# learningmatter-mit/surface-sampling

Measured on AMD Instinct MI355X. Metric: MC energy-evaluations/sec (SrTiO3(001) ~250-atom slabs, 3-model PaiNN ensemble E+F incl. neighbor list), higher is better.
Workload: dtype f32 via fp16x2-split MFMA (3 products), fp32 accumulate; neighbor decisions f64; 1 GPU; SrTiO3(001) PaiNN x3, 256 batched independent chains per GPU (BASELINE configs[3]), 248-272 atoms/chain; chains_per_gpu=256, atoms_per_gpu=66503, edges_per_gpu=2747786, slots_per_gpu=2836316, models=3, streams_per_gpu=2, parallelism=one GPU, no collective

## Files before the change

surface-sampling_amd/csrc/nbr.hip:

```cpp
#include "nbr_dev.h"

namespace vssr {

__global__ void k_wrap(int n, const double *__restrict__ pos, const int *__restrict__ atom_cfg,
                       const double *__restrict__ cell, const double *__restrict__ invcell,
                       const uint8_t *__restrict__ pbc, double *__restrict__ wpos, int *__restrict__ wrap) {
    int i = blockIdx.x * blockDim.x + threadIdx.x;
    if (i >= n) return;
    wrap_atom(i, pos, atom_cfg, cell, invcell, pbc, wpos, wrap);
}

template <bool FILL, int LPC>
__global__ void __launch_bounds__(256)
k_nbr(int n, const double *__restrict__ wpos, const int *__restrict__ atom_cfg,
      const int *__restrict__ cfg_start, const double *__restrict__ cell, const double *__restrict__ invcell,
      const int *__restrict__ nimg, double rc2, int *__restrict__ deg, const int *__restrict__ row_start, float4 *__restrict__ edge,
      int *__restrict__ edge_S, long long slot_cap, unsigned long long *__restrict__ hits_buf, int hits_stride,
      const unsigned char *__restrict__ active) {
    const int i = blockIdx.x * (256 / LPC) + threadIdx.x / LPC;
    if (i >= n) return;
    nbr_row<FILL, LPC>(i, wpos, atom_cfg, cfg_start, cell, invcell, nimg, rc2, deg, row_start, edge, edge_S, slot_cap, hits_buf, hits_stride,
                       active);
}

struct ScanTile {
    int d[4], pd[4], p, real;
};
__device__ __forceinline__ ScanTile scan_tile_load(int n, const int *__restrict__ deg, int i0) {
    ScanTile s;
    if (i0 + 3 < n) {
        const int4 v = *reinterpret_cast<const int4 *>(deg + i0);
        s.d[0] = v.x; s.d[1] = v.y; s.d[2] = v.z; s.d[3] = v.w;
    } else {
#pragma unroll
        for (int u = 0; u < 4; ++u) s.d[u] = i0 + u < n ? deg[i0 + u] : 0;
    }
#pragma unroll
    for (int u = 0; u < 4; ++u) s.pd[u] = i0 + u < n ? max((s.d[u] + 3) & ~3, 8) : 0;
    s.p = s.pd[0] + s.pd[1] + s.pd[2] + s.pd[3];
    s.real = s.d[0] + s.d[1] + s.d[2] + s.d[3];
    return s;
}

__global__ void __launch_bounds__(1024)
k_scan_tiles(int n, const int *__restrict__ deg, int *__restrict__ tile_sums ) {
    __shared__ int wsum[16], wreal[16];
    const int t = threadIdx.x, lane = t & 63, w = t >> 6;
    const ScanTile s = scan_tile_load(n, deg, blockIdx.x * 4096 + 4 * t);
    const int x = wave_incl_scan_i32(s.p), xr = wave_incl_scan_i32(s.real);
    if (lane == 63) { wsum[w] = x; wreal[w] = xr; }
    __syncthreads();
    if (t == 0) {
        int a = 0, b = 0;
#pragma unroll
        for (int k = 0; k < 16; ++k) { a += wsum[k]; b += wreal[k]; }
        tile_sums[2 * blockIdx.x] = a;
        tile_sums[2 * blockIdx.x + 1] = b;
    }
}

__global__ void __launch_bounds__(1024)
k_scan_rows(int n, const int *__restrict__ deg, int *__restrict__ row_start, int *__restrict__ counters,
            long long slot_cap, const int *__restrict__ tile_sums) {
    __shared__ int wsum[16], wreal[16];
    __shared__ long long wrun[16], wrun_real[16];
    const int t = threadIdx.x, lane = t & 63, w = t >> 6, tile = blockIdx.x;
    const bool last = tile == (int)gridDim.x - 1;
    long long run = 0, run_real = 0;
    for (int k = t; k < tile; k += 1024) {
        run += tile_sums[2 * k];
        if (last) run_real += tile_sums[2 * k + 1];
    }
#pragma unroll
    for (int o = 32; o > 0; o >>= 1) {
        run += __shfl_xor(run, o);
        run_real += __shfl_xor(run_real, o);
    }
    if (lane == 0) { wrun[w] = run; wrun_real[w] = run_real; }
    const ScanTile s = scan_tile_load(n, deg, tile * 4096 + 4 * t);
    const int x = wave_incl_scan_i32(s.p);
    if (lane == 63) wsum[w] = x;
    if (!tile_sums) {
        const int xr = wave_incl_scan_i32(s.real);
        if (lane == 63) wreal[w] = xr;
    }
    __syncthreads();
    run = 0; run_real = 0;
    int woff = 0;
#pragma unroll
    for (int k = 0; k < 16; ++k) {
        run += wrun[k];
        run_real += wrun_real[k];
        if (k < w) woff += wsum[k];
    }
    const int i0 = tile * 4096 + 4 * t;
    int o = (int)(run + woff + x - s.p);
#pragma unroll
    for (int u = 0; u < 4; ++u) {
        if (i0 + u < n) row_start[i0 + u] = o;
        o += s.pd[u];
    }
    if (last && t == 0) {
        long long own = 0, own_real = 0;
        if (tile_sums) { own = tile_sums[2 * tile]; own_real = tile_sums[2 * tile + 1]; }
        else {
            for (int k = 0; k < 16; ++k) { own += wsum[k]; own_real += wreal[k]; }
        }
        const long long total = run + own, total_real = run_real + own_real;
        row_start[n] = (int)total;
        counters[0] = (int)total;
        counters[1] = (int)total_real;
        counters[2] = (total > slot_cap - 64 || total > 2147483000LL) ? 1 : 0;
    }
}

template <int LPC>
__global__ void __launch_bounds__(256)
k_rev(int n, const int *__restrict__ row_start, const float4 *__restrict__ edge,
      const int *__restrict__ edge_S, int *__restrict__ rev, const int *__restrict__ counters, ActiveView av) {
    const int i = blockIdx.x * (256 / LPC) + threadIdx.x / LPC;
    if (i >= n || counters[2] || !av.atom(i)) return;
    rev_row<LPC>(i, row_start, edge, edge_S, rev);
}

__device__ __forceinline__ void split2_f16(float x, unsigned &h, unsigned &l) {
    const _Float16 hh = (_Float16)x;
    const _Float16 ll = (_Float16)(x - (float)hh);
    h = __builtin_bit_cast(unsigned short, hh);
    l = __builtin_bit_cast(unsigned short, ll);
}
__device__ __forceinline__ size_t f16_unit(size_t slot, int kq, int piece) {
    return (slot >> 2) * 32 + (size_t)piece * 16 + (size_t)kq * 4 + (slot & 3);
}
__device__ __forceinline__ void write_f16_record(const float (&v)[5], float env, uint4 *__restrict__ tab, size_t slot, int kq,
                                                 float spare, unsigned jbits) {
    unsigned h[6], l[6];
#pragma unroll
    for (int k = 0; k < 5; ++k) split2_f16(v[k], h[k], l[k]);
    split2_f16(env, h[5], l[5]);
    auto pk = [](unsigned lo, unsigned hi) { return lo | (hi << 16); };
    const unsigned env_piece = kq == 0 ? l[5] : kq == 3 ? 0u : h[5];
    tab[f16_unit(slot, kq, 0)] = make_uint4(pk(l[0], l[1]), pk(l[2], l[3]), pk(l[4], env_piece), pk(h[0], h[1]));
    tab[f16_unit(slot, kq, 1)] = make_uint4(pk(h[2], h[3]), pk(h[4], h[4]), __float_as_uint(spare), jbits);
}

__device__ __forceinline__ float quarter_class_sum(float x) {
    x += __builtin_bit_cast(float, __builtin_amdgcn_update_dpp(0, __builtin_bit_cast(int, x), 0x124, 0xF, 0xF, true));
    x += __builtin_bit_cast(float, __builtin_amdgcn_update_dpp(0, __builtin_bit_cast(int, x), 0x128, 0xF, 0xF, true));
    const unsigned u = __float_as_uint(x);
    const auto r32 = __builtin_amdgcn_permlane32_swap(u, u, false, false);
    const float y = __uint_as_float(r32[0]) + __uint_as_float(r32[1]);
    const unsigned v = __float_as_uint(y);
    const auto r16 = __builtin_amdgcn_permlane16_swap(v, v, false, false);
    return __uint_as_float(r16[0]) + __uint_as_float(r16[1]);
}

template <int NZ>
__global__ void __launch_bounds__(64) k_edge_geom(int n_atoms, const int *__restrict__ row_start, const int *__restrict__ atom_cfg,
                            const int *__restrict__ cfg_start, const float4 *__restrict__ edge,
                            const int *__restrict__ counters, float rc, float excl_sigma, int excl_power,
                            float4 *__restrict__ erec, float *__restrict__ rho,
                            float2 *__restrict__ dist2, uint4 *__restrict__ rho16, uint4 *__restrict__ drho16,
                            const int *__restrict__ Z, const int *__restrict__ zmap, unsigned char *__restrict__ zslot,
                            float *__restrict__ e_excl, const unsigned char *__restrict__ active, float *__restrict__ l0T) {
    if (counters[2]) return;
    float tacc[NZ > 0 ? NZ : 1][4][6];
#pragma unroll
    for (int z = 0; z < (NZ > 0 ? NZ : 1); ++z)
#pragma unroll
        for (int c = 0; c < 4; ++c)
#pragma unroll
            for (int k = 0; k < 6; ++k) tacc[z][c][k] = 0.f;
    const int i = blockIdx.x;
    if (active && !active[atom_cfg[i]]) return;
    const int a0 = cfg_start[atom_cfg[i]];
// ... 71 lines not shown
            float x = __uint_as_float(r16[0]) + __uint_as_float(r16[1]);
            x += __builtin_bit_cast(float, __builtin_amdgcn_update_dpp(0, __builtin_bit_cast(int, x), 0x128, 0xF, 0xF, true));
            x += __builtin_bit_cast(float, __builtin_amdgcn_update_dpp(0, __builtin_bit_cast(int, x), 0x124, 0xF, 0xF, true));
            quart[w] = x;
        }
        const int lane = threadIdx.x, rho = lane >> 4, kq = lane & 3;
        if ((lane & 12) == 0) {
#pragma unroll
            for (int b = 0; b < NZ; ++b) {
                const int zc = rho * NZ + b, z = zc >> 2, c = zc & 3;
                float2 *dst = reinterpret_cast<float2 *>(l0T + ((size_t)i * NZ + z) * 96 + c * 24 + kq * 6);
                dst[0] = make_float2(quart[6 * b], quart[6 * b + 1]);
                dst[1] = make_float2(quart[6 * b + 2], quart[6 * b + 3]);
                dst[2] = make_float2(quart[6 * b + 4], quart[6 * b + 5]);
            }
        }
    }
}

constexpr int BSORT_N = 2048;
__device__ __forceinline__ void lds_bitonic_sort(unsigned *keys) {
    for (int k = 2; k <= BSORT_N; k <<= 1)
        for (int j = k >> 1; j > 0; j >>= 1) {
            for (int t = threadIdx.x; t < BSORT_N / 2; t += blockDim.x) {
                const int i = 2 * t - (t & (j - 1)), l = i + j;
                const unsigned a = keys[i], b2 = keys[l];
                const bool up = (i & k) == 0;
                if ((a > b2) == up) { keys[i] = b2; keys[l] = a; }
            }
            __syncthreads();
        }
}

__global__ void __launch_bounds__(256)
k_bundle_sort(const int *__restrict__ cfg_start, const int *__restrict__ row_start, const int *__restrict__ counters,
              int4 *__restrict__ bundle, const unsigned char *__restrict__ active, int sort_keys) {
    extern __shared__ int sdeg[];
    if (counters[2] || (active && !active[blockIdx.x])) return;
    const int b = blockIdx.x, a0 = cfg_start[b], n = cfg_start[b + 1] - a0;
    for (int c = threadIdx.x; c < n; c += blockDim.x) sdeg[c] = row_start[a0 + c + 1] - row_start[a0 + c];
    __syncthreads();
    if (n <= BSORT_N && sort_keys) {
        unsigned *keys = reinterpret_cast<unsigned *>(sdeg) + n;
        for (int c = threadIdx.x; c < BSORT_N; c += blockDim.x) keys[c] = c < n ? ((unsigned)(4095 - min(sdeg[c], 4095)) << 11) | (unsigned)c : 0xFFFFFFFFu;
        __syncthreads();
        lds_bitonic_sort(keys);
        for (int r = threadIdx.x; r < n; r += blockDim.x) {
            const int c = (int)(keys[r] & 2047u);
            bundle[a0 + r] = make_int4(c, row_start[a0 + c], sdeg[c], 0);
        }
        return;
    }
    for (int c = threadIdx.x; c < n; c += blockDim.x) {
        const int d = sdeg[c];
        int rank = 0;
        for (int o = 0; o < n; ++o) {
            const int od = sdeg[o];
            rank += (od > d || (od == d && o < c)) ? 1 : 0;
        }
        bundle[a0 + rank] = make_int4(c, row_start[a0 + c], d, 0);
    }
}

__global__ void __launch_bounds__(1024)
k_bundle_sort_sub(const int *__restrict__ list, const int *__restrict__ cfg_start, const int *__restrict__ row_start,
                  const float4 *__restrict__ edge, const int *__restrict__ counters, int N, int n_cfg, int chunk_max,
                  int4 *__restrict__ bundle_sub, int *__restrict__ n_entries, const unsigned char *__restrict__ active) {
    extern __shared__ int sdeg[];
    const int b = list[blockIdx.x];
    if (counters[2] || (active && !active[b])) return;
    const int a0 = cfg_start[b], n = cfg_start[b + 1] - a0;
    const int P = sub_passes(n, chunk_max), chunk = sub_chunk(n, chunk_max);
    int *len = sdeg, *first = sdeg + SUB_MAX_PASSES * n;
    __shared__ int cnt[SUB_MAX_PASSES];
    if (threadIdx.x < SUB_MAX_PASSES) cnt[threadIdx.x] = 0;
    __syncthreads();
    const int lane = threadIdx.x & 15;
    for (int c = threadIdx.x >> 4; c < n; c += blockDim.x >> 4) {
        const int rs = row_start[a0 + c], re = row_start[a0 + c + 1];
        int below[SUB_MAX_PASSES];
#pragma unroll
        for (int p = 0; p < SUB_MAX_PASSES; ++p) below[p] = 0;
        for (int e = rs + lane; e < re; e += 16) {
            const int j = __float_as_int(edge[e].w);
            if (j < 0) continue;
            const int jl = j - a0;
#pragma unroll
            for (int p = 0; p < SUB_MAX_PASSES; ++p) below[p] += (p + 1 >= P || jl < (p + 1) * chunk) ? 1 : 0;
        }
#pragma unroll
        for (int p = 0; p < SUB_MAX_PASSES; ++p) {
            int x = below[p];
            x += __shfl_xor(x, 1); x += __shfl_xor(x, 2); x += __shfl_xor(x, 4); x += __shfl_xor(x, 8);
            below[p] = x;
        }
        if (lane == 0) {
            int kprev = 0;
            for (int p = 0; p < P; ++p) {
                const int k = below[p];
                const bool any = k > kprev;
                const int f = kprev & ~3, last = p + 1 < P ? min((k + 3) & ~3, re - rs) : re - rs;
                len[p * n + c] = any ? last - f : 0;
                first[p * n + c] = f;
                if (any && p > 0) atomicAdd(&cnt[p], 1);
                kprev = k;
            }
        }
    }
    __syncthreads();
    if (threadIdx.x >= 1 && threadIdx.x < SUB_MAX_PASSES) n_entries[(size_t)(threadIdx.x - 1) * n_cfg + b] = cnt[threadIdx.x];
    unsigned *keys = reinterpret_cast<unsigned *>(sdeg + 2 * SUB_MAX_PASSES * n);
    for (int p = 0; p < P; ++p) {
        const int *lp = len + p * n;
        __syncthreads();
        for (int c = threadIdx.x; c < BSORT_N; c += blockDim.x) keys[c] = c < n ? ((unsigned)(4095 - min(lp[c], 4095)) << 11) | (unsigned)c : 0xFFFFFFFFu;
        __syncthreads();
        lds_bitonic_sort(keys);
        for (int r = threadIdx.x; r < n; r += blockDim.x) {
            const int c = (int)(keys[r] & 2047u);
            bundle_sub[(size_t)p * N + a0 + r] = make_int4(c, row_start[a0 + c] + first[p * n + c], lp[c], 0);
        }
    }
}

int build_neighbors(vssr_handle *h, double cutoff) {
    const int n = h->n_atoms;
    hipStream_t st = h->stream;
    if (h->d_wpos.ensure(sizeof(double) * 3 * n) || h->d_wrap.ensure(sizeof(int) * 3 * n) ||
        h->d_deg.ensure(sizeof(int) * n) || h->d_row_start.ensure(sizeof(int) * (n + 1)) ||
        h->d_counters.ensure(sizeof(int) * 4) || h->d_tile_sums.ensure(sizeof(int) * 2 * ((size_t)n / 4096 + 1)))
        return set_err(h, VSSR_E_NOMEM, "neighbor buffers: out of device memory");
    if (h->slot_cap < (int64_t)n * h->cap_per_atom + 64) h->slot_cap = (int64_t)n * h->cap_per_atom + 64;
    if (h->d_edge.ensure(sizeof(float4) * h->slot_cap) || h->d_edge_S.ensure(sizeof(int) * h->slot_cap) ||
        h->d_rev.ensure(sizeof(int) * h->slot_cap))
        return set_err(h, VSSR_E_NOMEM, "edge buffers: out of device memory");
    unsigned long long *hits_buf = nullptr;
    const int hits_stride = (h->max_cfg_atoms + 63) & ~63;
    if (h->max_images <= 64 && (size_t)n * hits_stride * 8 <= ((size_t)1 << 30) &&
        !h->d_hits.ensure((size_t)n * hits_stride * 8))
        hits_buf = h->d_hits.as<unsigned long long>();
    h->prof.begin(KC_NBR, st);
    dim3 blk(128), grd((n + 127) / 128);
    const int lpc_rev = h->kind != Kind::PAINN ? 16 : 32;
    dim3 wblk(256);
    auto grid_for = [&](int lpc) { return dim3((n + 256 / lpc - 1) / (256 / lpc)); };
#define NBR_ARGS(FILLING) n, h->d_wpos.as<double>(), h->d_atom_cfg.as<int>(), h->d_cfg_start.as<int>(), h->d_cell.as<double>(),          \
        h->d_invcell.as<double>(), h->d_nimg.as<int>(), cutoff * cutoff, h->d_deg.as<int>(),                                            \
        (FILLING) ? h->d_row_start.as<int>() : (const int *)nullptr, (FILLING) ? h->d_edge.as<float4>() : (float4 *)nullptr,            \
        (FILLING) ? h->d_edge_S.as<int>() : (int *)nullptr, (FILLING) ? (long long)h->slot_cap : (long long)0, hits_buf, hits_stride,   \
        h->active_mask
    hipLaunchKernelGGL(k_wrap, grd, blk, 0, st, n, h->d_pos.as<double>(), h->d_atom_cfg.as<int>(),
                       h->d_cell.as<double>(), h->d_invcell.as<double>(), h->d_pbc.as<uint8_t>(),
                       h->d_wpos.as<double>(), h->d_wrap.as<int>());
    hipLaunchKernelGGL((k_nbr<false, 16>), grid_for(16), wblk, 0, st, NBR_ARGS(false));
    const int n_tiles = n > 0 ? (n + 4095) / 4096 : 1;
    if (n_tiles > 1)
        hipLaunchKernelGGL(k_scan_tiles, dim3(n_tiles), dim3(1024), 0, st, n, h->d_deg.as<int>(), h->d_tile_sums.as<int>());
    hipLaunchKernelGGL(k_scan_rows, dim3(n_tiles), dim3(1024), 0, st, n, h->d_deg.as<int>(),
                       h->d_row_start.as<int>(), h->d_counters.as<int>(), (long long)h->slot_cap,
                       n_tiles > 1 ? h->d_tile_sums.as<int>() : (const int *)nullptr);
    hipLaunchKernelGGL((k_nbr<true, 16>), grid_for(16), wblk, 0, st, NBR_ARGS(true));
#undef NBR_ARGS
    const ActiveView rev_av{h->active_mask, h->d_atom_cfg.as<int>()};
#define REV_ARGS n, h->d_row_start.as<int>(), h->d_edge.as<float4>(), h->d_edge_S.as<int>(), h->d_rev.as<int>(), h->d_counters.as<int>(), rev_av
    if (lpc_rev == 16) hipLaunchKernelGGL(k_rev<16>, grid_for(16), wblk, 0, st, REV_ARGS);
    else hipLaunchKernelGGL(k_rev<32>, grid_for(32), wblk, 0, st, REV_ARGS);
#undef REV_ARGS
    if (h->kind == Kind::PAINN && !h->painn_general) {
        const int nzf = (h->l0_enabled && h->l0_nz >= 1 && h->l0_nz <= 4) ? h->l0_nz : 0;
        const bool want_f32 = h->l0_enabled && nzf == 0;
        if ((want_f32 && (h->d_erec.ensure(sizeof(float4) * h->slot_cap) || h->d_rho.ensure(sizeof(float) * 24 * h->slot_cap))) ||
            h->d_dist.ensure(sizeof(float2) * h->slot_cap) ||
            h->d_rho16.ensure(sizeof(uint4) * 8 * h->slot_cap) || h->d_drho16.ensure(sizeof(uint4) * 8 * h->slot_cap) ||
            h->d_zslot.ensure((size_t)h->slot_cap) || h->d_bundle.ensure(sizeof(int4) * (size_t)n) ||
            h->d_excl.ensure(sizeof(float) * (size_t)n))
            return set_err(h, VSSR_E_NOMEM, "edge geometry tables: out of device memory");
        const void *tabs[2] = {h->d_rho16.as<uint4>(), h->d_drho16.as<uint4>()};
        bool cleared = h->zero_entry_cap == h->slot_cap;
        for (int k = 0; k < 2; ++k) cleared = cleared && h->zero_entry_tab[k] == tabs[k];
        if (!cleared) {
            VSSR_HIP(h, hipMemsetAsync(h->d_rho16.as<uint4>() + 32 * (size_t)((h->slot_cap >> 2) - 1), 0, 32 * sizeof(uint4), st));
            VSSR_HIP(h, hipMemsetAsync(h->d_drho16.as<uint4>() + 32 * (size_t)((h->slot_cap >> 2) - 1), 0, 32 * sizeof(uint4), st));
            h->zero_entry_cap = h->slot_cap;
            for (int k = 0; k < 2; ++k) h->zero_entry_tab[k] = tabs[k];
        }
        if (nzf && h->d_l0T.ensure(sizeof(float) * (size_t)n * nzf * 96))
            return set_err(h, VSSR_E_NOMEM, "layer-0 factorisation buffers: out of device memory");
        h->l0T_by_geom = nzf > 0;
#define LAUNCH_GEOM(NZ)                                                                                                          \
        hipLaunchKernelGGL(k_edge_geom<NZ>, dim3(n), dim3(64), 0, st, n, h->d_row_start.as<int>(), h->d_atom_cfg.as<int>(),      \
                           h->d_cfg_start.as<int>(), h->d_edge.as<float4>(), h->d_counters.as<int>(), h->cutoff,               \
                           h->excl_sigma, h->excl_power, want_f32 ? h->d_erec.as<float4>() : (float4 *)nullptr,                \
                           want_f32 ? h->d_rho.as<float>() : (float *)nullptr, h->d_dist.as<float2>(), h->d_rho16.as<uint4>(), \
                           h->d_drho16.as<uint4>(), h->d_Z.as<int>(), h->d_zmap.as<int>(), h->d_zslot.as<unsigned char>(),     \
                           h->d_excl.as<float>(), h->active_mask, nzf ? h->d_l0T.as<float>() : (float *)nullptr)
        switch (nzf) {
            case 1: LAUNCH_GEOM(1); break;
            case 2: LAUNCH_GEOM(2); break;
            case 3: LAUNCH_GEOM(3); break;
            case 4: LAUNCH_GEOM(4); break;
            default: LAUNCH_GEOM(0); break;
        }
#undef LAUNCH_GEOM
        if ((size_t)h->max_cfg_atoms * sizeof(int) <= 48 * 1024) {
            const int sort_keys = h->max_cfg_atoms > 512 && h->max_cfg_atoms <= BSORT_N;
            hipLaunchKernelGGL(k_bundle_sort, dim3(h->n_cfg), dim3(256),
                               (size_t)h->max_cfg_atoms * sizeof(int) + (sort_keys ? BSORT_N * sizeof(unsigned) : 0), st,
                               h->d_cfg_start.as<int>(), h->d_row_start.as<int>(), h->d_counters.as<int>(),
                               h->d_bundle.as<int4>(), h->active_mask, sort_keys);
            auto sub_tables = [&](vssr::DevBuf &buf, const int *list, int n_list, int max_atoms, int chunk) -> int {
                if (sub_passes(max_atoms, chunk) > SUB_MAX_PASSES) return set_err(h, VSSR_E_BADARG, "neighbor sub-range too small for this chain");
                if (buf.ensure(sizeof(int4) * SUB_MAX_PASSES * (size_t)n + sizeof(int) * (SUB_MAX_PASSES - 1) * (size_t)h->n_cfg))
                    return set_err(h, VSSR_E_NOMEM, "bundle tables: out of device memory");
                hipLaunchKernelGGL(k_bundle_sort_sub, dim3(n_list), dim3(1024),
                                   2 * SUB_MAX_PASSES * (size_t)max_atoms * sizeof(int) + BSORT_N * sizeof(unsigned), st, list,
                                   h->d_cfg_start.as<int>(), h->d_row_start.as<int>(), h->d_edge.as<float4>(), h->d_counters.as<int>(), n, h->n_cfg,
                                   chunk, buf.as<int4>(), reinterpret_cast<int *>(buf.as<int4>() + SUB_MAX_PASSES * (size_t)n), h->active_mask);
                return VSSR_OK;
            };
            if (h->fwd_two_pass && h->n_class[EDGE_CLASS_FS4] > 0) {
                int off = 0;
                for (int c = 0; c < EDGE_CLASS_FS4; ++c) off += h->n_class[c];
                const int rc2 = sub_tables(h->d_bundle_sub, h->d_class_list.as<int>() + off, h->n_class[EDGE_CLASS_FS4], h->max_class_atoms[EDGE_CLASS_FS4],
                                           h->sub_chunk_fwd ? h->sub_chunk_fwd : sub_chunk_max(h->fwd_two_pass));
                if (rc2) return rc2;
            }
            if (h->n_bclass[EDGE_BCLASS_FS16P] > 0) {
                int off = 0;
                for (int c = 0; c < EDGE_MFMA_CLASSES; ++c) off += h->n_class[c];
                for (int c = 0; c < EDGE_BCLASS_FS16P; ++c) off += h->n_bclass[c];
                const int rc2 = sub_tables(h->d_bundle_subb, h->d_class_list.as<int>() + off, h->n_bclass[EDGE_BCLASS_FS16P],
                                           h->max_bclass_atoms[EDGE_BCLASS_FS16P], h->sub_chunk_bwd ? h->sub_chunk_bwd : sub_chunk_max_bwd());
                if (rc2) return rc2;
            }
        }
    }
    h->prof.end(st);
    VSSR_HIP(h, hipMemcpyAsync(h->h_counters, h->d_counters.as<int>(), sizeof(int) * 4,
                               hipMemcpyDeviceToHost, st));
    return VSSR_OK;
}

}
```

surface-sampling_amd/csrc/nbr_dev.h:

```cpp
#ifndef VSSR_NBR_DEV_H
#define VSSR_NBR_DEV_H
#include "vssr_internal.h"

namespace vssr {

__device__ inline int pack_shift(int s0, int s1, int s2) {
    return ((s0 + 128) & 255) | (((s1 + 128) & 255) << 8) | (((s2 + 128) & 255) << 16);
}
__device__ inline void unpack_shift(int p, int &s0, int &s1, int &s2) {
    s0 = (p & 255) - 128;
    s1 = ((p >> 8) & 255) - 128;
    s2 = ((p >> 16) & 255) - 128;
}

__device__ __forceinline__ void wrap_atom(int i, const double *__restrict__ pos, const int *__restrict__ atom_cfg,
                                          const double *__restrict__ cell, const double *__restrict__ invcell,
                                          const uint8_t *__restrict__ pbc, double *__restrict__ wpos, int *__restrict__ wrap) {
    int c = atom_cfg[i];
    const double *C = cell + 9 * c, *I = invcell + 9 * c;
    double p[3] = {pos[3 * i], pos[3 * i + 1], pos[3 * i + 2]};
    double q[3] = {p[0], p[1], p[2]};
    for (int a = 0; a < 3; ++a) {
        int w = 0;
        if (pbc[3 * c + a]) {
            double f = I[3 * a] * p[0] + I[3 * a + 1] * p[1] + I[3 * a + 2] * p[2];
            w = (int)floor(f);
            q[0] -= w * C[3 * a];
            q[1] -= w * C[3 * a + 1];
            q[2] -= w * C[3 * a + 2];
        }
        wrap[3 * i + a] = w;
    }
    wpos[3 * i] = q[0];
    wpos[3 * i + 1] = q[1];
    wpos[3 * i + 2] = q[2];
}

template <int LPC>
__device__ __forceinline__ int group_excl_scan(int v, int &total) {
    if constexpr (LPC == 64) {
        const int x = wave_incl_scan_i32(v);
        total = __builtin_amdgcn_readlane(x, 63);
        return x - v;
    } else {
        static_assert(LPC == 16 || LPC == 32, "a wave, half a wave or one 16-lane row per centre");
        int x = v;
        x += __builtin_amdgcn_update_dpp(0, x, 0x111, 0xF, 0xF, true);
        x += __builtin_amdgcn_update_dpp(0, x, 0x112, 0xF, 0xF, true);
        x += __builtin_amdgcn_update_dpp(0, x, 0x114, 0xF, 0xF, true);
        x += __builtin_amdgcn_update_dpp(0, x, 0x118, 0xF, 0xF, true);
        if constexpr (LPC == 32) x += __builtin_amdgcn_update_dpp(0, x, 0x142, 0xA, 0xF, false);
        total = __shfl(x, (threadIdx.x & 63) | (LPC - 1));
        return x - v;
    }
}

template <bool FILL, int LPC>
__device__ __forceinline__ void nbr_row(int i, const double *__restrict__ wpos, const int *__restrict__ atom_cfg,
      const int *__restrict__ cfg_start, const double *__restrict__ cell, const double *__restrict__ invcell,
      const int *__restrict__ nimg, double rc2, int *__restrict__ deg, const int *__restrict__ row_start, float4 *__restrict__ edge,
      int *__restrict__ edge_S, long long slot_cap, unsigned long long *__restrict__ hits_buf, int hits_stride,
      const unsigned char *__restrict__ active) {
    const int lane = threadIdx.x & (LPC - 1);
    const int c = atom_cfg[i];
    if (active && !active[c]) {
        if (!FILL && lane == 0) deg[i] = 0;
        return;
    }
    const int a0 = cfg_start[c], a1 = cfg_start[c + 1];
    const double *C = cell + 9 * c;
    const int n0 = nimg[3 * c], n1 = nimg[3 * c + 1], n2 = nimg[3 * c + 2];
    const double C0 = C[0], C1 = C[1], C2 = C[2], C3 = C[3], C4 = C[4], C5 = C[5], C6 = C[6], C7 = C[7], C8 = C[8];
    const double px = wpos[3 * i], py = wpos[3 * i + 1], pz = wpos[3 * i + 2];
    const double *I = invcell + 9 * c;
    const double I0 = I[0], I1 = I[1], I2 = I[2], I3 = I[3], I4 = I[4], I5 = I[5], I6 = I[6], I7 = I[7], I8 = I[8];
    const double rcut = sqrt(rc2);
    const double wd0 = rcut * sqrt(I0 * I0 + I1 * I1 + I2 * I2) * (1.0 + 1e-9) + 1e-9;
    const double wd1 = rcut * sqrt(I3 * I3 + I4 * I4 + I5 * I5) * (1.0 + 1e-9) + 1e-9;
    const double wd2 = rcut * sqrt(I6 * I6 + I7 * I7 + I8 * I8) * (1.0 + 1e-9) + 1e-9;
    long long base = FILL ? (long long)row_start[i] : 0;
    int run = 0;
    for (int j0 = a0; j0 < a1; j0 += LPC) {
        const int j = j0 + lane;
        const bool have = j < a1;
        double bx = 0, by = 0, bz = 0;
        if (have) { bx = wpos[3 * j] - px; by = wpos[3 * j + 1] - py; bz = wpos[3 * j + 2] - pz; }
        int cnt = 0;
        unsigned long long hits = 0ull;
        unsigned long long *hslot = hits_buf ? hits_buf + (size_t)i * hits_stride + (j - a0) : nullptr;
        if (FILL && hslot) {
            if (have) {
                hits = *hslot;
                cnt = __builtin_popcountll(hits);
            }
        } else if (have) {
            const double f0 = I0 * bx + I1 * by + I2 * bz, f1 = I3 * bx + I4 * by + I5 * bz, f2 = I6 * bx + I7 * by + I8 * bz;
            const int lo0 = n0 ? max(-n0, (int)ceil(-wd0 - f0)) : 0, hi0 = n0 ? min(n0, (int)floor(wd0 - f0)) : 0;
            const int lo1 = n1 ? max(-n1, (int)ceil(-wd1 - f1)) : 0, hi1 = n1 ? min(n1, (int)floor(wd1 - f1)) : 0;
            const int lo2 = n2 ? max(-n2, (int)ceil(-wd2 - f2)) : 0, hi2 = n2 ? min(n2, (int)floor(wd2 - f2)) : 0;
            const int iw1 = 2 * n1 + 1, iw2 = 2 * n2 + 1;
            for (int s0 = lo0; s0 <= hi0; ++s0)
                for (int s1 = lo1; s1 <= hi1; ++s1)
                    for (int s2 = lo2; s2 <= hi2; ++s2) {
                        const int img = ((s0 + n0) * iw1 + (s1 + n1)) * iw2 + (s2 + n2);
                        if (i == j && s0 == 0 && s1 == 0 && s2 == 0) continue;
                        double rx = bx + s0 * C0 + s1 * C3 + s2 * C6;
                        double ry = by + s0 * C1 + s1 * C4 + s2 * C7;
                        double rz = bz + s0 * C2 + s1 * C5 + s2 * C8;
                        double d2 = rx * rx + ry * ry + rz * rz;
                        if (d2 <= rc2 && d2 > 0.0) {
                            ++cnt;
                            if (img < 64) hits |= 1ull << img;
                        }
                    }
            if (!FILL && hslot) *hslot = hits;
        }
        int total;
        const int off = group_excl_scan<LPC>(cnt, total);
        if (FILL && cnt > 0) {
            long long slot = base + run + off;
            const int w1 = 2 * n1 + 1, w2 = 2 * n2 + 1;
            if ((2 * n0 + 1) * w1 * w2 <= 64) {
                while (hits) {
                    const int img = __builtin_ctzll(hits);
                    hits &= hits - 1;
                    const int s0 = img / (w1 * w2) - n0, s1 = (img / w2) % w1 - n1, s2 = img % w2 - n2;
                    const double rx = bx + s0 * C0 + s1 * C3 + s2 * C6;
                    const double ry = by + s0 * C1 + s1 * C4 + s2 * C7;
                    const double rz = bz + s0 * C2 + s1 * C5 + s2 * C8;
                    if (slot < slot_cap) {
                        edge[slot] = make_float4((float)rx, (float)ry, (float)rz, __int_as_float(j));
                        edge_S[slot] = pack_shift(s0, s1, s2);
                    }
                    ++slot;
                }
            } else {
                for (int s0 = -n0; s0 <= n0; ++s0)
                    for (int s1 = -n1; s1 <= n1; ++s1)
                        for (int s2 = -n2; s2 <= n2; ++s2) {
                            if (i == j && s0 == 0 && s1 == 0 && s2 == 0) continue;
                            double rx = bx + s0 * C0 + s1 * C3 + s2 * C6;
                            double ry = by + s0 * C1 + s1 * C4 + s2 * C7;
                            double rz = bz + s0 * C2 + s1 * C5 + s2 * C8;
                            double d2 = rx * rx + ry * ry + rz * rz;
                            if (d2 > rc2 || d2 <= 0.0) continue;
                            if (slot < slot_cap) {
                                edge[slot] = make_float4((float)rx, (float)ry, (float)rz, __int_as_float(j));
                                edge_S[slot] = pack_shift(s0, s1, s2);
                            }
                            ++slot;
                        }
            }
        }
        run += total;
    }
    if (FILL) {
        const int padded = max((run + 3) & ~3, 8);
        const long long slot = base + run + lane;
        if (lane < padded - run && slot < slot_cap) {
            edge[slot] = make_float4(0.f, 0.f, 0.f, __int_as_float(-1));
            edge_S[slot] = pack_shift(0, 0, 0);
        }
    } else if (lane == 0) {
        deg[i] = run;
    }
}

template <int LPC>
__device__ __forceinline__ void rev_row(int i, const int *__restrict__ row_start, const float4 *__restrict__ edge,
                                        const int *__restrict__ edge_S, int *__restrict__ rev) {
    const int lane = threadIdx.x & (LPC - 1);
    for (int e = row_start[i] + lane; e < row_start[i + 1]; e += LPC) {
        int j = __float_as_int(edge[e].w);
        int found = -1;
        if (j >= 0) {
            int s0, s1, s2;
            unpack_shift(edge_S[e], s0, s1, s2);
            const int want = pack_shift(-s0, -s1, -s2);
            int lo = row_start[j], hi = row_start[j + 1];
            const int row_end = hi;
            while (lo < hi) {
                const int mid = (lo + hi) >> 1;
                const int jm = __float_as_int(edge[mid].w);
                if (jm >= 0 && jm < i) lo = mid + 1; else hi = mid;
            }
            for (int e2 = lo; e2 < row_end && __float_as_int(edge[e2].w) == i; ++e2)
                if (edge_S[e2] == want) {
                    found = e2;
                    break;
                }
        }
        rev[e] = found;
    }
}

}
#endif
```

surface-sampling_amd/csrc/vssr_internal.h:

```cpp
#pragma once

#include <hip/hip_runtime.h>

#include <cstdint>
#include <cstdio>
#include <cstdlib>
#include <cstring>
#include <memory>
#include <string>
#include <utility>
#include <vector>

#include "../../include/vssr_eval.h"

namespace vssr {

constexpr int F = 128;
constexpr int F3 = 3 * F;
constexpr int MAX_LAYERS = 4;
constexpr int MAX_MODELS = 8;
constexpr int RB_MAX = 24;
constexpr int NODE_TILE = 8;
constexpr int L0_MAX_SPECIES = 8;

// ... 162 lines not shown
    OwnedStream &operator=(const OwnedStream &) = delete;
    ~OwnedStream() { if (s) (void)hipStreamDestroy(s); }
    operator hipStream_t() const { return s; }
};
struct PinnedInts {
    int *p = nullptr;
    PinnedInts() = default;
    PinnedInts(const PinnedInts &) = delete;
    PinnedInts &operator=(const PinnedInts &) = delete;
    ~PinnedInts() { if (p) (void)hipHostFree(p); }
    operator int *() const { return p; }
};

enum KernelClass {
    KC_NBR = 0,
    KC_EMBED,
    KC_MSG_MLP,
    KC_EDGE_FWD,
    KC_UPDATE_FWD,
    KC_READOUT,
    KC_UPDATE_BWD,
    KC_EDGE_BWD,
    KC_MSG_MLP_BWD,
    KC_FINALIZE,
    KC_ANALYTIC,
    KC_L0_FWD,
    KC_L0_BWD,
    KC_NEB_PROJECT,
    KC_NEB_STEP,
    KC_COUNT
};
extern const char *const kKernelClassNames[KC_COUNT];

struct Profiler {
    bool enabled = false;
    struct Rec { int kc; hipEvent_t a, b; };
    std::vector<Rec> pending;
    std::vector<hipEvent_t> pool;
    int64_t launches[KC_COUNT] = {0};
    double total_ms[KC_COUNT] = {0};
    hipEvent_t get_event();
    void begin(int kc, hipStream_t s);
    void end(hipStream_t s);
    void collect();
    void reset();
    Profiler() = default;
    Profiler(const Profiler &) = delete;
    Profiler &operator=(const Profiler &) = delete;
    ~Profiler();
};

struct GmmFit {
    int cov_type = 0;
    int init = 0;
    int max_iter = 100, n_init = 1;
    double tol = 1e-3, reg_covar = 1e-6;
    uint64_t seed = 0;
    bool device_ready = false, fitted = false;
    int64_t n = 0, cap = 0;
    DevBuf rows;
    double *x() const { return rows.as<double>(); }
    std::vector<double> i_means, i_weights, i_prec;
    std::vector<int> i_labels;
    bool has_means = false, has_weights = false, has_prec = false, has_labels = false;
    DevBuf resp, labels, lbpart, status, flags;
    DevBuf part_s, part_q, part_n, nk, means, avg_x2, w, cov, part_cov, chol_w, chol_y, centers, assign_part;
    DevBuf b_w, b_means, b_cov, b_P, b_c, b_kc, b_mask;
};

struct Cluster {
    int n_components = 0, whiten = 1, d_clu = 3, d_pad = 3;
    bool pca_done = false;
    int64_t n_pts = 0;
    DevBuf mean, denom, part_sum, part_cov, cov, evec, eval, comp, comp_t, ev, ratio, jac, xr;
    DevBuf pts;
    DevBuf cen[2], siz[2], cid[2];
    DevBuf nn, flag, blk, rec, counters;
};

enum class Kind : int {
    NONE = 0,
    PAINN = 1,
    TERSOFF = 2,
    EAM = 3,
    SW = 4,
    GMM = 5,
    GMM_FIT = 6,
    CLUSTER = 7,
    PAIR = 8,
    VASHISHTA = 9,
    COUNT
};
constexpr unsigned kind_bit(Kind k) { return 1u << (int)k; }
constexpr unsigned KINDS_EVAL = kind_bit(Kind::PAINN) | kind_bit(Kind::TERSOFF) | kind_bit(Kind::EAM) | kind_bit(Kind::SW) |
                                kind_bit(Kind::PAIR) | kind_bit(Kind::VASHISHTA);

}

struct vssr_handle {
    vssr::Kind kind = vssr::Kind::NONE;
    vssr_eam_grid eam_grid = {0, 0, 0.0, 0.0, 0.0};
    int eam_nel = 0, eam_fs = 0;
    bool eam_adp = false;
    double vash_r0max = 0.0;
    int device = 0;
    vssr::OwnedStream stream;
    std::string err;
    vssr::Profiler prof;

    int edge_impl = 1;
    int max_cfg_atoms = 0;
    vssr::DevBuf d_chain_class, d_class_list;
    int n_class[5] = {0, 0, 0, 0, 0}, max_class_atoms[5] = {0, 0, 0, 0, 0};
    int n_bclass[5] = {0, 0, 0, 0, 0}, max_bclass_atoms[5] = {0, 0, 0, 0, 0};
    int fs16_max_atoms = -1, fs8_max_atoms = -1;
    int max_images = 0;

    int n_models = 0, n_rbf = 20, num_conv = 3, n_embed = 100, readout_hidden = 64;
    int feat_dim = vssr::F;
    bool painn_general = false;
    float cutoff = 5.f;
    int excl_vol = 1, excl_power = 12;
    float excl_sigma = 1.5f;
    double units_per_ev = 1.0;
    bool has_offset = false;
    double offset_const = 0.0;

    vssr::DevBuf weights;
    vssr::DevBuf wd16;
    vssr::DevBuf node16;
    vssr::DevBuf model_table;
    vssr::DevBuf offset_per_z;

    int n_types = 0;
    double pot_cutoff = 0;
    bool ew_on = false;
    double ew_g = 0, ew_kcut = 0, ew_q[8] = {0, 0, 0, 0, 0, 0, 0, 0};
    int ew_stride = 0;
    vssr::DevBuf d_ew_S;
    vssr::DevBuf pot_params;

    bool batch_valid = false, ran = false;
    int n_cfg = 0, n_atoms = 0;
    std::vector<int> h_n_atoms, h_cfg_start;
    vssr::DevBuf d_pos, d_wpos, d_wrap, d_Z, d_atom_cfg, d_cfg_start, d_cell, d_invcell, d_nimg, d_pbc;
    vssr::DevBuf d_deg, d_row_start, d_edge, d_edge_S, d_rev, d_counters, d_tile_sums;
    vssr::DevBuf d_erec, d_rho, d_dist, d_rho16, d_drho16, d_zslot, d_bundle, d_excl;
    vssr::DevBuf d_bundle_sub;
    int bwd_multi_pass = 1;
    int sub_chunk_fwd = 0, sub_chunk_bwd = 0;
    vssr::DevBuf d_bundle_subb;
    int fwd_two_pass = 16;
    vssr::DevBuf d_hits;
    int l0_enabled = 1, l0_nz = 0;
    bool l0_used = false;
    vssr::DevBuf d_l0A, d_l0At;
    vssr::DevBuf d_zmap, d_zlist;
    vssr::DevBuf d_l0T, d_l0Q;
    vssr::DevBuf d_opt_state, d_opt_vec, d_bfgs_q, d_bfgs_b, d_fixed, d_relax_steps, d_relax_conv, d_active;
    const unsigned char *active_mask = nullptr;
    int relax_regrows = 0;
    long long relax_lockstep = 0;
    int relax_compactions = 0;
    vssr::DevBuf d_cmp;
    vssr::DevBuf d_cm;
    long long relax_chain_evals = 0;
    int traj_interval = 0, traj_records = 0, traj_B = 0, traj_N = 0;
    vssr::DevBuf d_traj_pos, d_traj_f, d_traj_e, d_traj_n;
    bool graph_partial = false;
    bool l0T_by_geom = false;
    int64_t zero_entry_cap = -1;
    const void *zero_entry_tab[2] = {nullptr, nullptr};
    int cap_per_atom = 64;
    int cm_cap_per_atom = 0;
    int cg_driver = 0;
    int cg_last_driver = 0;
    bool cap_tight = false;
    vssr::DevBuf d_md_vel;
    vssr::DevBuf d_md_aux;
    bool md_vel_valid = false;
    int md_driver = 0;
    int md_last_driver = 0;
    vssr::DevBuf d_vib;
    vssr::DevBuf d_neb;
    uint32_t last_want = 0;
    int64_t slot_cap = 0;
    vssr::PinnedInts h_counters;

    vssr::DevBuf d_state;
    vssr::StateView sv;
    vssr::DevBuf d_gbar;
    vssr::DevBuf d_upd_save;
    vssr::DevBuf d_gpart;
    int debug_keep = 0;
    int upd_save = 0;
    vssr::DevBuf d_energy, d_energy_std, d_energy_models, d_forces, d_forces_std, d_e_atoms;
    vssr::DevBuf d_energy64;
    vssr::DevBuf d_pot_e, d_pot_ea, d_pot_f;
    vssr::DevBuf d_sat, d_sat_out;
    std::vector<unsigned> h_sat;
    bool h_sat_valid = false;
    vssr::DevBuf d_stress;

    int gmm_K = 0, gmm_D = 0, gmm_Dp = 0;
    double gmm_log2pi = 0.0;
    vssr::DevBuf d_gmm_P;
    vssr::DevBuf d_gmm_c;
    vssr::DevBuf d_gmm_kc;
    vssr::DevBuf d_gmm_mask;
    vssr::DevBuf d_gmm_x, d_gmm_lp, d_gmm_nll, d_gmm_sys, d_gmm_start;
    std::unique_ptr<vssr::GmmFit> fit;
    std::unique_ptr<vssr::Cluster> clu;
};

namespace vssr {

int set_err(vssr_handle *h, int code, const char *fmt, ...);
#define VSSR_HIP(h, expr)                                                                    \
    do {                                                                                     \
        hipError_t _e = (expr);                                                              \
        if (_e != hipSuccess)                                                                \
            return vssr::set_err(h, VSSR_E_DEVICE, "%s failed: %s (%s:%d)", #expr,          \
                                 hipGetErrorString(_e), __FILE__, __LINE__);                 \
    } while (0)

int check_kind(vssr_handle *h, unsigned served, const char *func);
int device_in_range(vssr_handle *h, int device);
int open_device(vssr_handle *h, int device);
void publish_create_error(const vssr_handle *h);
template <class Init>
int create_handle(Kind kind, int device, vssr_handle **out, Init init, bool range_check = true) {
    vssr_handle *h = new vssr_handle();
    h->kind = kind;
    int rc = range_check ? device_in_range(h, device) : VSSR_OK;
    if (!rc) rc = open_device(h, device);
    if (!rc) rc = init(h);
    if (rc) {
        publish_create_error(h);
        vssr_destroy(h);
        return rc;
    }
    *out = h;
    return VSSR_OK;
}
int run_any(vssr_handle *h, uint32_t want);
int sync_and_check(vssr_handle *h);
int grow_slot_cap(vssr_handle *h);

int build_neighbors(vssr_handle *h, double cutoff);
int painn_alloc_state(vssr_handle *h);
int painn_run(vssr_handle *h, uint32_t want);
int painn_stress(vssr_handle *h);
int painn_alloc_results(vssr_handle *h);
void painn_finalize(vssr_handle *h, const GraphView &G, uint32_t want);
GraphView graph_view(const vssr_handle *h);
int painn_gen_upload(vssr_handle *h, const vssr_painn_config *cfg);
int painn_gen_run(vssr_handle *h, uint32_t want);
int tersoff_run(vssr_handle *h, uint32_t want);
int eam_run(vssr_handle *h, uint32_t want);
int adp_run(vssr_handle *h, uint32_t want);
int adp_stress(vssr_handle *h);
int sw_run(vssr_handle *h, uint32_t want);
int pair_run(vssr_handle *h, uint32_t want);
int vashishta_run(vssr_handle *h, uint32_t want);
int gmm_upload(vssr_handle *g, const double *means, const double *prec_chol, const double *weights);
int gmm_score_f64(vssr_handle *g, hipStream_t st, int64_t n, const double *x_dev);
int gmm_score_f32(vssr_handle *g, hipStream_t st, int64_t n, const float *x_dev);
int gmm_mean_rows(vssr_handle *g, hipStream_t st, int B, const int *start, const float *emb);
int gmm_reduce(vssr_handle *g, hipStream_t st, int B, const int *start, int order);
int gmm_fit_check_config(const vssr_gmm_fit_config *cfg);
int gmm_fit_append_host(vssr_handle *h, int64_t n_rows, const double *x);
int gmm_fit_append_f32(vssr_handle *h, hipStream_t st, int64_t n_rows, const float *emb_dev);
int gmm_fit_append_f64p(vssr_handle *h, hipStream_t st, int64_t n_rows, const double *x_dev);
int gmm_fit_set_init(vssr_handle *h, const double *means, const double *weights, const double *precisions, const int32_t *labels);
int gmm_fit_run(vssr_handle *h, vssr_gmm_fit_result *res);
int gmm_fit_params(vssr_handle *h, double *weights, double *means, double *covariances, double *prec_chol);
int gmm_fit_copy_scorer(vssr_handle *h, vssr_handle *g);
int gmm_fit_centered_cov(vssr_handle *h, hipStream_t st, const double *X, int n, int D, int Dp, const double *mean, const double *denom,
                         DevBuf &part, double *cov);
int cluster_pca(vssr_handle *h, vssr_cluster_pca_result *res);
int cluster_pca_params(vssr_handle *h, double *mean, double *components, double *explained_variance, double *ratio);
int cluster_projected(vssr_handle *h, int64_t first, int64_t n_rows, double *xr);
int cluster_set_points(vssr_handle *h, int64_t n, const double *pts);
int cluster_linkage(vssr_handle *h, double *Z, int32_t *n_rounds);
int cluster_pad_dims(int d);
int tersoff_stress(vssr_handle *h);
int eam_stress(vssr_handle *h);
int sw_stress(vssr_handle *h);
struct PotView;
void ewald_run(vssr_handle *h, const PotView &V);
int ewald_stress(vssr_handle *h);
int pair_stress(vssr_handle *h);
int vashishta_stress(vssr_handle *h);
struct Evaluator {
    bool f64;
    int (*run)(vssr_handle *h, uint32_t want);
    int (*stress)(vssr_handle *h);
    double (*cutoff)(const vssr_handle *h);
};
const Evaluator &evaluator(const vssr_handle *h);
inline bool is_analytic(const vssr_handle *h) { return evaluator(h).f64; }
void eam_build_spline(const double *f, int n, double delta, double *spl );
int relax_fire(vssr_handle *h, const vssr_fire_params &p, const uint8_t *fixed_host, uint32_t want);
int relax_bfgs(vssr_handle *h, const vssr_bfgs_params &p, const uint8_t *fixed_host, uint32_t want);
int relax_begin(vssr_handle *h, const uint8_t *fixed_host, int steps_ints_per_chain, const uint8_t *&fixed);
int relax_regrow(vssr_handle *h, int cap, long long &it, int window);
int relax_cg(vssr_handle *h, const vssr_cg_params *cp, const uint8_t *fixed_host, uint32_t want);
int relax_bfgsls(vssr_handle *h, const vssr_bfgsls_params *bp, const uint8_t *fixed_host, uint32_t want);
bool chain_min_supported(const vssr_handle *h);
int chain_min_cg(vssr_handle *h, const vssr_cg_params *cp, const uint8_t *fixed_host, uint32_t want);
int node_mfma_init(vssr_handle *h);
void launch_msg_mlp_mfma(hipStream_t st, int N, int M, int l, const ActiveView &av, const ModelW *MW, const float *s_in,
                         float *phi);
void launch_msg_mlp_bwd_mfma(hipStream_t st, int N, int M, int l, const ActiveView &av, const ModelW *MW, const float *s_in,
                             const float *phibar, const float *sbar_msg, float *sbar_in);
void launch_update_fwd_mfma(hipStream_t st, int N, int M, int l, const ActiveView &av, const ModelW *MW, const float *s_msg,
                            const float *v_msg, float *s_out, float *v_out, float *phi_next, void *save);
size_t update_save_bytes(int N, int M);
bool readout_mfma_supported(int hidden);
void launch_readout_mfma(hipStream_t st, int N, int M, const ActiveView &av, const ModelW *MW, const float *s, const float *e_excl,
                         float *e_atom);
void launch_update_bwd_mfma(hipStream_t st, int N, int M, int l, int mode, int vbar_is_zero, const ActiveView &av, const ModelW *MW,
                            const float *s_msg, const float *v_msg, const float *sbar_src, const float *vbar,
                            const float *s_next, const float *phibar, const float *e_excl, float *e_atom,
                            float *sbar_msg, float *vbar_msg, float *s_last, const void *save);
void pack_mfma_tiles16(const float *Wsrc, int rows, int K, unsigned *dst );
void build_wd16(const float *Wd, const float *bd, unsigned *dst );
void l0_build_tables(const float *blob_embed, const float *W1, const float *b1, const float *W2, const float *b2,
                     const float *Wd, const float *bd, int n_embed, float *A, float *At);
void l0_pack_tables(const float *A, int n_embed, unsigned *A16, unsigned *At16);
size_t l0_packed_dwords(int n_embed);
int l0_mfma_init(vssr_handle *h);
int l0_run_forward(vssr_handle *h, const GraphView &G, float *s_msg, float *v_msg);
int l0_run_reverse(vssr_handle *h, const GraphView &G, int first_write, int fresh_mfma, const float *sbar_msg, const float *vbar_msg,
                   float4 *gbar);
int edge_mfma_init(vssr_handle *h);
enum { EDGE_CLASS_FS16 = 0, EDGE_CLASS_FS16M = 1, EDGE_CLASS_FS8 = 2, EDGE_CLASS_FS4 = 3, EDGE_CLASS_GATHER = 4, EDGE_CLASSES = 5,
       EDGE_MFMA_CLASSES = 4 };
enum { EDGE_BCLASS_FS16 = 0, EDGE_BCLASS_FS8 = 1, EDGE_BCLASS_FS4 = 2, EDGE_BCLASS_FS16P = 3, EDGE_BCLASS_GATHER = 4, EDGE_BCLASSES = 5,
       EDGE_MFMA_BCLASSES = 4 };
__host__ __device__ constexpr int edge_bclass_slices(int c) { return (c == EDGE_BCLASS_FS16 || c == EDGE_BCLASS_FS16P) ? 8 : c == EDGE_BCLASS_FS8 ? 16 : c == EDGE_BCLASS_FS4 ? 32 : 1; }
int edge_bclass_of(int n_atoms);
int edge_class_of(int n_atoms);
constexpr int SUB_MAX_PASSES = 4;
__host__ __device__ constexpr int sub_chunk_max(int width) { return width == 16 ? 400 : 784; }
__host__ __device__ constexpr int sub_chunk_max_bwd() { return 550; }
__host__ __device__ constexpr int sub_passes(int n_atoms, int chunk_max) { return (n_atoms + chunk_max - 1) / chunk_max; }
__host__ __device__ constexpr int sub_chunk(int n_atoms, int chunk_max) { return (n_atoms + sub_passes(n_atoms, chunk_max) - 1) / sub_passes(n_atoms, chunk_max); }
int edge_class_groups(int cls);
void launch_edge_bwd_mfma(hipStream_t st, int cls, int N, const int *list, int n_list, int M, int l, int max_atoms,
                          const ModelW *MW, const GraphView &G, const int *counters, int zero_slot,
                          const float *v_in, const float *phi, const float *sbar_msg, const float *vbar_msg,
                          float *phibar, float *vbar_in, float *gpart, long long slot_cap, int n_groups, int group_off,
                          const int4 *bundle_sub, int sub_chunk);
void launch_edge_fwd_mfma(hipStream_t st, int cls, int N, const int *list, int n_list, int M, int l, int max_atoms, const ModelW *MW,
                          const GraphView &G, const int *counters, int zero_slot, const float *s_in, const float *v_in,
                          const float *phi, float *s_msg, float *v_msg, const int4 *bundle_sub, int sub_width, int sub_chunk);

}
```

Measured before the change: 24780 evaluations/s.

## Fill neighbor edges and reverse indices in one pass from stored hit prefixes

The counting pass now stores, next to each per-pair image hit mask, the exclusive prefix offset of that pair within its row. A new flat fill kernel uses these words to write edge vectors, shift codes and reverse-edge indices directly, one wave per atom. This replaces the separate fill kernel and the reverse-index kernel, so pair distances are not recomputed and no reverse search is needed. It only applies when the hits buffer exists and the image and atom limits hold, and it adds a second random read per pair to find the mirror entry.

```diff
diff --git a/surface-sampling_amd/csrc/nbr.hip b/surface-sampling_amd/csrc/nbr.hip
--- a/surface-sampling_amd/csrc/nbr.hip
+++ b/surface-sampling_amd/csrc/nbr.hip
@@ -10,7 +10,7 @@
     wrap_atom(i, pos, atom_cfg, cell, invcell, pbc, wpos, wrap);
 }
 
-template <bool FILL, int LPC>
+template <bool FILL, int LPC, bool PFX = false>
 __global__ void __launch_bounds__(256)
 k_nbr(int n, const double *__restrict__ wpos, const int *__restrict__ atom_cfg,
       const int *__restrict__ cfg_start, const double *__restrict__ cell, const double *__restrict__ invcell,
@@ -19,8 +19,66 @@
       const unsigned char *__restrict__ active) {
     const int i = blockIdx.x * (256 / LPC) + threadIdx.x / LPC;
     if (i >= n) return;
-    nbr_row<FILL, LPC>(i, wpos, atom_cfg, cfg_start, cell, invcell, nimg, rc2, deg, row_start, edge, edge_S, slot_cap, hits_buf, hits_stride,
-                       active);
+    nbr_row<FILL, LPC, PFX>(i, wpos, atom_cfg, cfg_start, cell, invcell, nimg, rc2, deg, row_start, edge, edge_S, slot_cap, hits_buf,
+                            hits_stride, active);
+}
+
+__global__ void __launch_bounds__(256)
+k_nbr_flat(int n, const double *__restrict__ wpos, const int *__restrict__ atom_cfg, const int *__restrict__ cfg_start,
+           const double *__restrict__ cell, const int *__restrict__ nimg, const int *__restrict__ deg,
+           const int *__restrict__ row_start, float4 *__restrict__ edge, int *__restrict__ edge_S, int *__restrict__ rev,
+           long long slot_cap, const unsigned long long *__restrict__ hits_buf, int hits_stride,
+           const int *__restrict__ counters, const unsigned char *__restrict__ active) {
+    const int i = __builtin_amdgcn_readfirstlane(blockIdx.x * 4 + (threadIdx.x >> 6));
+    if (i >= n || counters[2]) return;
+    const int c = atom_cfg[i];
+    if (active && !active[c]) return;
+    const int lane = threadIdx.x & 63;
+    const int a0 = cfg_start[c], nc = cfg_start[c + 1] - a0, il = i - a0;
+    const double *C = cell + 9 * c;
+    const int n0 = nimg[3 * c], n1 = nimg[3 * c + 1], n2 = nimg[3 * c + 2];
+    const int w1 = 2 * n1 + 1, w2 = 2 * n2 + 1, W = (2 * n0 + 1) * w1 * w2;
+    const double C0 = C[0], C1 = C[1], C2 = C[2], C3 = C[3], C4 = C[4], C5 = C[5], C6 = C[6], C7 = C[7], C8 = C[8];
+    const double px = wpos[3 * i], py = wpos[3 * i + 1], pz = wpos[3 * i + 2];
+    const long long base = row_start[i];
+    const unsigned long long *row = hits_buf + (size_t)i * hits_stride;
+    unsigned long long next = lane < nc ? row[lane] : 0ull;
+    for (int jl = lane; jl < nc; jl += 64) {
+        const unsigned long long w = next;
+        next = jl + 64 < nc ? row[jl + 64] : 0ull;
+        unsigned long long hits = w & NBR_MASK48;
+        if (!hits) continue;
+        const int j = a0 + jl;
+        const unsigned long long wr = hits_buf[(size_t)j * hits_stride + il];
+        const unsigned long long rmask = wr & NBR_MASK48;
+        const long long rbase = (long long)row_start[j] + (long long)(wr >> 48);
+        const double bx = wpos[3 * j] - px, by = wpos[3 * j + 1] - py, bz = wpos[3 * j + 2] - pz;
+        long long slot = base + (long long)(w >> 48);
+        while (hits) {
+            const int img = __builtin_ctzll(hits);
+            hits &= hits - 1;
+            const int s0 = img / (w1 * w2) - n0, s1 = (img / w2) % w1 - n1, s2 = img % w2 - n2;
+            const double rx = bx + s0 * C0 + s1 * C3 + s2 * C6;
+            const double ry = by + s0 * C1 + s1 * C4 + s2 * C7;
+            const double rz = bz + s0 * C2 + s1 * C5 + s2 * C8;
+            const int mir = W - 1 - img;
+            const int r = ((rmask >> mir) & 1ull) ? (int)(rbase + __builtin_popcountll(rmask & ((1ull << mir) - 1))) : -1;
+            if (slot < slot_cap) {
+                edge[slot] = make_float4((float)rx, (float)ry, (float)rz, __int_as_float(j));
+                edge_S[slot] = pack_shift(s0, s1, s2);
+                rev[slot] = r;
+            }
+            ++slot;
+        }
+    }
+    const int run = deg[i];
+    const int padded = max((run + 3) & ~3, 8);
+    const long long slot = base + run + lane;
+    if (lane < padded - run && slot < slot_cap) {
+        edge[slot] = make_float4(0.f, 0.f, 0.f, __int_as_float(-1));
+        edge_S[slot] = pack_shift(0, 0, 0);
+        rev[slot] = -1;
+    }
 }
 
 struct ScanTile {
@@ -398,20 +456,29 @@
     hipLaunchKernelGGL(k_wrap, grd, blk, 0, st, n, h->d_pos.as<double>(), h->d_atom_cfg.as<int>(),
                        h->d_cell.as<double>(), h->d_invcell.as<double>(), h->d_pbc.as<uint8_t>(),
                        h->d_wpos.as<double>(), h->d_wrap.as<int>());
-    hipLaunchKernelGGL((k_nbr<false, 16>), grid_for(16), wblk, 0, st, NBR_ARGS(false));
+    const bool flat = hits_buf && !h->nbr_fill_replay && h->max_images <= 48 && (long long)h->max_cfg_atoms * h->max_images <= 65535;
+    if (flat) hipLaunchKernelGGL((k_nbr<false, 16, true>), grid_for(16), wblk, 0, st, NBR_ARGS(false));
+    else hipLaunchKernelGGL((k_nbr<false, 16>), grid_for(16), wblk, 0, st, NBR_ARGS(false));
     const int n_tiles = n > 0 ? (n + 4095) / 4096 : 1;
     if (n_tiles > 1)
         hipLaunchKernelGGL(k_scan_tiles, dim3(n_tiles), dim3(1024), 0, st, n, h->d_deg.as<int>(), h->d_tile_sums.as<int>());
     hipLaunchKernelGGL(k_scan_rows, dim3(n_tiles), dim3(1024), 0, st, n, h->d_deg.as<int>(),
                        h->d_row_start.as<int>(), h->d_counters.as<int>(), (long long)h->slot_cap,
                        n_tiles > 1 ? h->d_tile_sums.as<int>() : (const int *)nullptr);
-    hipLaunchKernelGGL((k_nbr<true, 16>), grid_for(16), wblk, 0, st, NBR_ARGS(true));
+    if (flat) {
+        hipLaunchKernelGGL(k_nbr_flat, grid_for(64), wblk, 0, st, n, h->d_wpos.as<double>(), h->d_atom_cfg.as<int>(), h->d_cfg_start.as<int>(),
+                           h->d_cell.as<double>(), h->d_nimg.as<int>(), h->d_deg.as<int>(), h->d_row_start.as<int>(), h->d_edge.as<float4>(),
+                           h->d_edge_S.as<int>(), h->d_rev.as<int>(), (long long)h->slot_cap, hits_buf, hits_stride, h->d_counters.as<int>(),
+                           h->active_mask);
+    } else {
+        hipLaunchKernelGGL((k_nbr<true, 16>), grid_for(16), wblk, 0, st, NBR_ARGS(true));
+        const ActiveView rev_av{h->active_mask, h->d_atom_cfg.as<int>()};
+#define REV_ARGS n, h->d_row_start.as<int>(), h->d_edge.as<float4>(), h->d_edge_S.as<int>(), h->d_rev.as<int>(), h->d_counters.as<int>(), rev_av
+        if (lpc_rev == 16) hipLaunchKernelGGL(k_rev<16>, grid_for(16), wblk, 0, st, REV_ARGS);
+        else hipLaunchKernelGGL(k_rev<32>, grid_for(32), wblk, 0, st, REV_ARGS);
+#undef REV_ARGS
+    }
 #undef NBR_ARGS
-    const ActiveView rev_av{h->active_mask, h->d_atom_cfg.as<int>()};
-#define REV_ARGS n, h->d_row_start.as<int>(), h->d_edge.as<float4>(), h->d_edge_S.as<int>(), h->d_rev.as<int>(), h->d_counters.as<int>(), rev_av
-    if (lpc_rev == 16) hipLaunchKernelGGL(k_rev<16>, grid_for(16), wblk, 0, st, REV_ARGS);
-    else hipLaunchKernelGGL(k_rev<32>, grid_for(32), wblk, 0, st, REV_ARGS);
-#undef REV_ARGS
     if (h->kind == Kind::PAINN && !h->painn_general) {
         const int nzf = (h->l0_enabled && h->l0_nz >= 1 && h->l0_nz <= 4) ? h->l0_nz : 0;
         const bool want_f32 = h->l0_enabled && nzf == 0;
diff --git a/surface-sampling_amd/csrc/nbr_dev.h b/surface-sampling_amd/csrc/nbr_dev.h
--- a/surface-sampling_amd/csrc/nbr_dev.h
+++ b/surface-sampling_amd/csrc/nbr_dev.h
@@ -55,12 +55,14 @@
     }
 }
 
-template <bool FILL, int LPC>
+constexpr unsigned long long NBR_MASK48 = (1ull << 48) - 1;
+template <bool FILL, int LPC, bool PFX = false>
 __device__ __forceinline__ void nbr_row(int i, const double *__restrict__ wpos, const int *__restrict__ atom_cfg,
       const int *__restrict__ cfg_start, const double *__restrict__ cell, const double *__restrict__ invcell,
       const int *__restrict__ nimg, double rc2, int *__restrict__ deg, const int *__restrict__ row_start, float4 *__restrict__ edge,
       int *__restrict__ edge_S, long long slot_cap, unsigned long long *__restrict__ hits_buf, int hits_stride,
       const unsigned char *__restrict__ active) {
+    static_assert(!(FILL && PFX), "the prefix words are written by the counting pass and read by k_nbr_flat only");
     const int lane = threadIdx.x & (LPC - 1);
     const int c = atom_cfg[i];
     if (active && !active[c]) {
@@ -113,10 +115,13 @@
                             if (img < 64) hits |= 1ull << img;
                         }
                     }
-            if (!FILL && hslot) *hslot = hits;
+            if constexpr (!PFX)
+                if (!FILL && hslot) *hslot = hits;
         }
         int total;
         const int off = group_excl_scan<LPC>(cnt, total);
+        if constexpr (PFX)
+            if (have) *hslot = hits | ((unsigned long long)(run + off) << 48);
         if (FILL && cnt > 0) {
             long long slot = base + run + off;
             const int w1 = 2 * n1 + 1, w2 = 2 * n2 + 1;
diff --git a/surface-sampling_amd/csrc/vssr_internal.h b/surface-sampling_amd/csrc/vssr_internal.h
--- a/surface-sampling_amd/csrc/vssr_internal.h
+++ b/surface-sampling_amd/csrc/vssr_internal.h
@@ -338,6 +338,7 @@
     vssr::DevBuf d_bundle_subb;
     int fwd_two_pass = 16;
     vssr::DevBuf d_hits;
+    bool nbr_fill_replay = false;
     int l0_enabled = 1, l0_nz = 0;
     bool l0_used = false;
     vssr::DevBuf d_l0A, d_l0At;
@@ -418,6 +419,7 @@
 int create_handle(Kind kind, int device, vssr_handle **out, Init init, bool range_check = true) {
     vssr_handle *h = new vssr_handle();
     h->kind = kind;
+    if (const char *e = getenv("VSSR_NBR_FILL")) h->nbr_fill_replay = strcmp(e, "replay") == 0;
     int rc = range_check ? device_in_range(h, device) : VSSR_OK;
     if (!rc) rc = open_device(h, device);
     if (!rc) rc = init(h);
```

After: 24900 evaluations/s, median of 6. About the same (+0.5%).
